# GT-RIPL/robo-vln

Measured on AMD Instinct MI355X. Metric: policy env-steps/sec (batched act()) at 256x256 RGB-D, 80-tok instr, higher is better.
Workload: dtype fp16 (range-calibrated fp16 storage and MFMA in BERT, both trunks and the cross-modal block; fp32 accumulate, fp32 recurrent state; DESIGN.md section 5); 1 GPU; BASELINE.json configs[1]: full HCM act() (hi->argmax->lo), 256x256 RGB-D, L=80, VLA N=1, LSTM-512; per_gpu_batch=64, global_batch=64, parallelism=single GPU

## Files before the change

include/hcm.h:

```cpp
#ifndef HCM_H
#define HCM_H

#include <stdint.h>

#ifdef __cplusplus
extern "C" {
#endif

typedef struct hcm_ctx* hcm_handle;

enum hcm_status {
    HCM_OK = 0,
    HCM_ERR_ARG = -1,
    HCM_ERR_STATE = -2,
    HCM_ERR_KEY = -3,
    HCM_ERR_SHAPE = -4,
    HCM_ERR_HIP = -5,
    HCM_ERR_UNSUPPORTED = -6,
    HCM_ERR_NOMEM = -7
};

enum hcm_dtype { HCM_F32 = 0, HCM_BF16 = 1, HCM_I32 = 2, HCM_I64 = 3, HCM_U8 = 4, HCM_F16 = 5 };
enum hcm_model { HCM_HIGH = 0, HCM_LOW = 1, HCM_CMA = 2 ,
                 HCM_S2S = 3  };
// ... 134 lines not shown
    int32_t struct_size;
    int32_t precision;
    int32_t max_batch;
    int32_t rgb_h, rgb_w, depth_h, depth_w;
    int32_t instr_len;
    int32_t vocab_size, embedding_size, instr_hidden;
    int32_t instr_rnn;
    int32_t bidirectional;
    int32_t rgb_encoder, depth_encoder;
    int32_t rgb_out, depth_out, depth_baseplanes;
    int32_t hidden, rnn_type;
    int32_t num_actions;
    int32_t num_sub_tasks;
    int32_t use_prev_action;
    int32_t is_bert;
    int32_t progress_monitor;
    int32_t ablate_instruction;
    int32_t ablate_depth;
    int32_t ablate_rgb;
    int32_t reserved[6];
} hcm_s2s_config;

int hcm_s2s_create(const hcm_s2s_config* cfg, hcm_handle* out);

int hcm_s2s_forward(hcm_handle h, const void* rgb, int rgb_dtype, const float* depth, const void* ids, int ids_dtype, int B, int B_instr, int L,
                    const float* h_in, const float* mask, float* out, float* stop, float* progress, float* h_out, void* stream);
int hcm_s2s_forward_seq(hcm_handle h, const void* rgb, int rgb_dtype, const float* depth, const void* ids, int ids_dtype, int T, int N, int B_instr,
                        int L, const float* h_in, const float* masks, float* out, float* stop, float* progress, float* h_out, void* stream);


int hcm_debug_enable_taps(hcm_handle h, int enable);
int hcm_debug_get_tap(hcm_handle h, const char* name, float* host_out, int64_t capacity,
                      int64_t* n_out, int64_t* shape_out);
int hcm_debug_igemm_prof(uint64_t* out8, int reset);
int hcm_debug_gemm256_prof(uint64_t* out1024, int reset);
int hcm_debug_marks(hcm_handle h, uint64_t* out256, char* names, int names_cap);

int hcm_op_conv2d(const void* x, const void* w_ohwi, const float* bias, const void* residual, void* y,
                  int dtype, int B, int H, int W, int Cin, int Cout, int KH, int KW, int stride, int pad,
                  int act, void* stream);
int hcm_op_conv2d_gn(const void* x, const void* w_ohwi, const float* gamma, const float* beta, const void* residual, void* y,
                     int dtype, int B, int H, int W, int Cin, int Cout, int KH, int KW, int stride, int pad, int groups, float eps,
                     int relu, void* stream);
int hcm_op_bottleneck_tail(const void* x, const void* w2, const float* b2, const void* w3, const float* b3, const void* identity,
                           void* y, int dtype, int B, int H, int W, int C1, int stride, void* stream);
int hcm_op_bottleneck_tail_next(const void* x, const void* w2, const float* b2, const void* w3, const float* b3, const void* identity,
                                void* y, const void* w1, const float* b1, void* o1, int dtype, int B, int H, int W, int C1, int stride,
                                int CN, void* stream);
int hcm_op_bottleneck_tail_ds(const void* x, const void* w2, const float* b2, const void* w3ds, const float* b3ds, const void* xd,
                              void* y, const void* w1, const float* b1, void* o1, int dtype, int B, int H, int W, int stride,
                              void* stream);
int hcm_op_conv2d_gn_large(const void* x, const void* w_ohwi, const float* gamma, const float* beta, const void* residual, void* y,
                           int dtype, int B, int H, int W, int Cin, int Cout, int KH, int KW, int stride, int pad, int groups, float eps,
                           int relu, void* stream);
int hcm_op_stem_conv(const void* x, int x_dtype, const void* w, const float* bias, void* y, int dtype, int B, int H, int W, int C,
                     int Cout, int KH, int KW, int stride, int pad, int K, int Kp, int rowrun, float scale, int act, void* stream);
int hcm_op_stem_conv_packed(const void* x, int x_dtype, const void* w, const float* bias, void* y, int dtype, int B, int H, int W,
                            int Cout, float scale, int act, void* scratch, void* stream);
int hcm_op_stem_conv_packed_pool(const void* x, int x_dtype, const void* w, const float* bias, void* y, int dtype, int B, int H, int W,
                                 int Cout, float scale, void* scratch, void* half_map, void* stream);
int hcm_op_stem_pool_fused(const void* x, int x_dtype, const void* w, const float* bias, void* y, int dtype, int B, int H, int W,
                           int Cout, float scale, void* scratch, void* stream);
int hcm_op_stem_pool_fused_red(const void* x, int x_dtype, const void* w, const float* bias, void* y, int dtype, int B, int H, int W,
                               int Cout, float scale, void* scratch, const void* w1, const float* b1, void* o1, void* stream);
int64_t hcm_op_stem_scratch_bytes(int B, int H, int W);
int hcm_op_depth_conv8x8s4(const float* depth, const void* w, const float* bias, void* y, int dtype, int B, int H, int act, void* scratch,
                           void* stream);
int hcm_op_simplecnn3(const float* depth, const void* w0, const float* b0, const void* w1_frag, const float* b1, const void* w2_frag, const float* b2,
                      void* y, int dtype, int B, int H, void* stream);
int hcm_op_linear(const void* x, const void* w, const float* bias, const void* residual, void* y,
                  int dtype, int M, int N, int K, int act, int out_f32, void* stream);
int hcm_op_vla_layer(const void* q, const void* I, const void* const* kv, const int* Lk, const void* const* att, void* const* out, float* const* pooled,
                     int ld_pool, const void* wo, const float* bo, const void* w1, const float* b1, const void* w2, const float* b2, const float* g1,
                     const float* be1, const float* g2, const float* be2, const int32_t* lens, int dtype, int B, int L, int d_ff, int streams,
                     void* stream);
int hcm_op_vla_layer_frag(const void* q, const void* I, const void* const* kv, const int* Lk, const void* const* att, void* const* out,
                          float* const* pooled, int ld_pool, const void* wo_frag, const float* bo, const void* w1_frag, const float* b1,
                          const void* w2_frag, const float* b2, const float* g1, const float* be1, const float* g2, const float* be2,
                          const int32_t* lens, int dtype, int B, int L, int d_ff, int streams, void* stream);
int hcm_op_linear_impl(const void* x, const void* w, const float* bias, const void* residual, void* y,
                       int dtype, int M, int N, int K, int act, int out_f32, int impl, void* stream);
int hcm_op_attention(const void* q, const void* k, const void* v, void* out, int dtype,
                     int B, int heads, int Lq, int Lk, int ldq, int ldk, int ldv, int ldo, void* stream);
int hcm_op_layernorm(const void* x, const void* residual, const float* gamma, const float* beta,
                     void* y, int dtype, int rows, int D, float eps, void* stream);
int hcm_op_pack_frag(const void* w, void* out, int dtype, int N, int K, void* stream);
int hcm_op_bert_attn_block(const void* qkv, const void* wo_frag, const float* bo, const void* residual, const float* residual32, const float* gamma,
                           const float* beta, void* y, float* y32, int dtype, int B, int L, const int32_t* lengths, float eps, void* stream);
int hcm_op_layernorm_post(const void* x, const void* residual, const float* gamma, const float* beta, const float* post, int post_rows,
                          void* y, int dtype, int rows, int D, float eps, void* stream);
int hcm_op_groupnorm(void* x_inplace, const void* residual, const float* gamma, const float* beta,
                     int dtype, int B, int HW, int C, int groups, float eps, int relu, void* stream);
int hcm_op_conv2d_gn_pool(const void* x, const void* w_ohwi, const float* gamma, const float* beta, void* y, int dtype, int B, int H, int W, int Cin,
                          int Cout, int KH, int KW, int stride, int pad, int groups, float eps, void* stream);
int hcm_op_conv2d_gn_res2(const void* x, const void* w_ohwi, const float* gamma, const float* beta, const void* x2, const void* w2_ohwi, const float* gamma2,
                          const float* beta2, void* y, int dtype, int B, int H, int W, int Cin, int Cin2, int stride2, int Cout, int groups, float eps,
                          int relu, void* stream);
int hcm_op_maxpool3x3s2(const void* x, void* y, int dtype, int B, int H, int W, int C, void* stream);
int hcm_op_val_loss(const float* logits, const float* vel, const float* stop, const int64_t* oracle_subtask, const float* corrected_actions,
                    const float* oracle_stop, float* result, int rows, int A, int num_sub_tasks, void* stream);

#ifdef __cplusplus
}
#endif
#endif
```

robo-vln_amd/_lib.py:

```python
import ctypes as C
import os

_HERE = os.path.dirname(os.path.abspath(__file__))
LIB_PATH = os.path.join(_HERE, "libhcm_dev.so" if os.environ.get("HCM_DEV_LIB", "0") not in ("", "0") else "libhcm.so")

HCM_F32, HCM_BF16, HCM_I32, HCM_I64, HCM_U8, HCM_F16 = 0, 1, 2, 3, 4, 5
HCM_HIGH, HCM_LOW, HCM_CMA, HCM_S2S = 0, 1, 2, 3
HCM_ENC_RESNET, HCM_ENC_SIMPLECNN = 0, 1
HCM_LSTM, HCM_GRU = 0, 1
(HCM_NUM_RECURRENT_LAYERS, HCM_HIDDEN_SIZE, HCM_NUM_ACTIONS, HCM_RECORD_WIDTH, HCM_WORKSPACE_BYTES,
 HCM_WEIGHT_BYTES, HCM_MAX_BATCH, HCM_GRAPH_LAUNCHES, HCM_EAGER_LAUNCHES, HCM_FP16_FALLBACK, HCM_CALIB_MAX_BERT, HCM_CALIB_MAX_DEPTH,
 HCM_CALIB_NONFINITE, HCM_CALIB_MAX_RGB, HCM_CALIB_MAX_VLA, HCM_STEP_NONFINITE, HCM_RANGE_FOLD, HCM_GATHER_JOINED) = range(18)
PRECISIONS = {"fp32": HCM_F32, "fp16": HCM_F16, "bf16": HCM_BF16}
ACT_NONE, ACT_RELU, ACT_GELU = 0, 1, 2
HCM_ACT_REUSE_INSTRUCTION = 1
HCM_ACT_HOST_FRAMES = 2
HCM_ACT_CHAIN_GRAPHS = 4

STATUS_EXC = {-1: ValueError, -2: RuntimeError, -3: KeyError, -4: ValueError, -5: RuntimeError, -6: ValueError,
              -7: MemoryError}


class HcmConfigStruct(C.Structure):
    _fields_ = [(n, C.c_int32) for n in (
# ... 4 lines not shown
        "bert_layers", "bert_hidden", "bert_heads", "bert_inter", "bert_vocab", "bert_max_pos",
        "build_high", "build_low", "use_prev_action", "ablate_instruction", "progress_monitor", "ablate_depth", "ablate_rgb")] + [("reserved", C.c_int32 * 8)]


class HcmCmaConfigStruct(C.Structure):
    _fields_ = [(n, C.c_int32) for n in (
        "struct_size", "precision", "max_batch", "rgb_h", "rgb_w", "depth_h", "depth_w", "instr_len",
        "vocab_size", "embedding_size", "instr_hidden", "bidirectional", "rgb_out", "depth_out", "depth_baseplanes",
        "hidden", "rnn_type", "num_actions", "use_prev_action", "rcm_state_encoder", "progress_monitor",
        "instr_rnn", "ablate_instruction", "ablate_depth", "ablate_rgb")] + [("reserved", C.c_int32 * 4)]


class HcmS2sConfigStruct(C.Structure):
    _fields_ = [(n, C.c_int32) for n in (
        "struct_size", "precision", "max_batch", "rgb_h", "rgb_w", "depth_h", "depth_w", "instr_len",
        "vocab_size", "embedding_size", "instr_hidden", "instr_rnn", "bidirectional", "rgb_encoder", "depth_encoder",
        "rgb_out", "depth_out", "depth_baseplanes", "hidden", "rnn_type", "num_actions", "num_sub_tasks",
        "use_prev_action", "is_bert", "progress_monitor", "ablate_instruction", "ablate_depth", "ablate_rgb")] + [("reserved", C.c_int32 * 6)]


EXPORTS = {
    "hcm_s2s_create": (C.c_int, [C.POINTER(HcmS2sConfigStruct), C.POINTER(C.c_void_p)]),
    "hcm_s2s_forward": (C.c_int, [C.c_void_p, C.c_void_p, C.c_int, C.c_void_p, C.c_void_p, C.c_int, C.c_int, C.c_int, C.c_int,
                                  C.c_void_p, C.c_void_p, C.c_void_p, C.c_void_p, C.c_void_p, C.c_void_p, C.c_void_p]),
    "hcm_s2s_forward_seq": (C.c_int, [C.c_void_p, C.c_void_p, C.c_int, C.c_void_p, C.c_void_p, C.c_int, C.c_int, C.c_int, C.c_int, C.c_int,
                                      C.c_void_p, C.c_void_p, C.c_void_p, C.c_void_p, C.c_void_p, C.c_void_p, C.c_void_p]),
    "hcm_cma_create": (C.c_int, [C.POINTER(HcmCmaConfigStruct), C.POINTER(C.c_void_p)]),
    "hcm_cma_forward": (C.c_int, [C.c_void_p, C.c_void_p, C.c_int, C.c_void_p, C.c_void_p, C.c_int, C.c_int, C.c_int,
                                  C.c_void_p, C.c_void_p, C.c_void_p, C.c_void_p, C.c_void_p, C.c_void_p]),
    "hcm_create": (C.c_int, [C.POINTER(HcmConfigStruct), C.POINTER(C.c_void_p)]),
    "hcm_load_tensor": (C.c_int, [C.c_void_p, C.c_int, C.c_char_p, C.c_void_p, C.c_int, C.POINTER(C.c_int64), C.c_int]),
    "hcm_finalize": (C.c_int, [C.c_void_p]),
    "hcm_high_forward": (C.c_int, [C.c_void_p, C.c_void_p, C.c_int, C.c_void_p, C.c_void_p, C.c_int, C.c_void_p, C.c_int, C.c_int,
                                   C.c_void_p, C.c_void_p, C.c_void_p, C.c_void_p, C.c_void_p]),
    "hcm_low_forward": (C.c_int, [C.c_void_p, C.c_void_p, C.c_int, C.c_void_p, C.c_int, C.c_void_p, C.c_void_p,
                                  C.c_void_p, C.c_void_p, C.c_void_p, C.c_void_p, C.c_void_p]),
    "hcm_high_forward_seq": (C.c_int, [C.c_void_p, C.c_void_p, C.c_int, C.c_void_p, C.c_void_p, C.c_int, C.c_void_p, C.c_int, C.c_int, C.c_int,
                                       C.c_void_p, C.c_void_p, C.c_void_p, C.c_void_p, C.c_void_p]),
    "hcm_low_forward_seq": (C.c_int, [C.c_void_p, C.c_void_p, C.c_int, C.c_void_p, C.c_int, C.c_int, C.c_void_p, C.c_void_p,
                                      C.c_void_p, C.c_void_p, C.c_void_p, C.c_void_p, C.c_void_p]),
    "hcm_val_step": (C.c_int, [C.c_void_p, C.c_void_p, C.c_int, C.c_void_p, C.c_void_p, C.c_int, C.c_void_p, C.c_int, C.c_int, C.c_int,
                               C.c_void_p, C.c_void_p, C.c_void_p, C.c_void_p, C.c_void_p, C.c_void_p, C.c_void_p, C.c_void_p, C.c_void_p,
                               C.c_void_p, C.c_void_p, C.c_void_p, C.c_void_p]),
    "hcm_act": (C.c_int, [C.c_void_p, C.c_void_p, C.c_int, C.c_void_p, C.c_void_p, C.c_int, C.c_void_p, C.c_int, C.c_int,
                          C.c_void_p, C.c_void_p, C.c_void_p, C.c_void_p, C.c_void_p, C.c_void_p, C.c_void_p]),
    "hcm_act_ex": (C.c_int, [C.c_void_p, C.c_void_p, C.c_int, C.c_void_p, C.c_void_p, C.c_int, C.c_void_p, C.c_int, C.c_int,
                             C.c_void_p, C.c_void_p, C.c_void_p, C.c_void_p, C.c_void_p, C.c_void_p, C.c_int, C.c_void_p]),
    "hcm_comm_unique_id": (C.c_int, [C.c_void_p]),
    "hcm_comm_init": (C.c_int, [C.c_void_p, C.c_void_p, C.c_int, C.c_int]),
    "hcm_comm_abort": (C.c_int, [C.c_void_p]),
    "hcm_gather_poison": (C.c_int, [C.c_void_p, C.c_int, C.c_void_p, C.c_void_p, C.c_void_p]),
    "hcm_act_gather": (C.c_int, [C.c_void_p, C.c_void_p, C.c_int, C.c_void_p, C.c_void_p, C.c_int, C.c_void_p, C.c_int, C.c_int,
                                 C.c_void_p, C.c_void_p, C.c_void_p, C.c_void_p, C.c_void_p, C.c_void_p, C.c_int, C.c_void_p, C.c_void_p]),
    "hcm_refresh_instruction": (C.c_int, [C.c_void_p, C.c_void_p, C.c_int, C.c_void_p, C.c_int, C.c_int, C.POINTER(C.c_int32), C.c_int, C.c_void_p]),
    "hcm_calibrate": (C.c_int, [C.c_void_p, C.c_void_p, C.c_int, C.c_void_p, C.c_void_p, C.c_int, C.c_int, C.c_int, C.c_void_p]),
    "hcm_release_host_weights": (C.c_int, [C.c_void_p]),
    "hcm_query": (C.c_int, [C.c_void_p, C.c_int, C.POINTER(C.c_int64)]),
    "hcm_guard_poll": (C.c_int, [C.c_void_p, C.c_void_p, C.POINTER(C.c_int64)]),
    "hcm_last_error": (C.c_char_p, [C.c_void_p]),
    "hcm_destroy": (None, [C.c_void_p]),
    "hcm_debug_enable_taps": (C.c_int, [C.c_void_p, C.c_int]),
    "hcm_debug_get_tap": (C.c_int, [C.c_void_p, C.c_char_p, C.c_void_p, C.c_int64, C.POINTER(C.c_int64), C.POINTER(C.c_int64)]),
    "hcm_debug_igemm_prof": (C.c_int, [C.POINTER(C.c_uint64), C.c_int]),
    "hcm_debug_gemm256_prof": (C.c_int, [C.POINTER(C.c_uint64), C.c_int]),
    "hcm_debug_marks": (C.c_int, [C.c_void_p, C.POINTER(C.c_uint64), C.c_char_p, C.c_int]),
    "hcm_op_conv2d": (C.c_int, [C.c_void_p] * 5 + [C.c_int] * 11 + [C.c_void_p]),
    "hcm_op_bottleneck_tail": (C.c_int, [C.c_void_p] * 7 + [C.c_int] * 6 + [C.c_void_p]),
    "hcm_op_bottleneck_tail_next": (C.c_int, [C.c_void_p] * 10 + [C.c_int] * 7 + [C.c_void_p]),
    "hcm_op_bottleneck_tail_ds": (C.c_int, [C.c_void_p] * 10 + [C.c_int] * 5 + [C.c_void_p]),
    "hcm_op_conv2d_gn": (C.c_int, [C.c_void_p] * 6 + [C.c_int] * 11 + [C.c_float, C.c_int, C.c_void_p]),
    "hcm_op_conv2d_gn_large": (C.c_int, [C.c_void_p] * 6 + [C.c_int] * 11 + [C.c_float, C.c_int, C.c_void_p]),
    "hcm_op_stem_conv": (C.c_int, [C.c_void_p, C.c_int, C.c_void_p, C.c_void_p, C.c_void_p] + [C.c_int] * 13 + [C.c_float, C.c_int, C.c_void_p]),
    "hcm_op_stem_conv_packed": (C.c_int, [C.c_void_p, C.c_int, C.c_void_p, C.c_void_p, C.c_void_p] + [C.c_int] * 5 + [C.c_float, C.c_int, C.c_void_p, C.c_void_p]),
    "hcm_op_stem_pool_fused": (C.c_int, [C.c_void_p, C.c_int, C.c_void_p, C.c_void_p, C.c_void_p] + [C.c_int] * 5 + [C.c_float, C.c_void_p, C.c_void_p]),
    "hcm_op_stem_pool_fused_red": (C.c_int, [C.c_void_p, C.c_int, C.c_void_p, C.c_void_p, C.c_void_p] + [C.c_int] * 5 + [C.c_float] + [C.c_void_p] * 5),
    "hcm_op_stem_conv_packed_pool": (C.c_int, [C.c_void_p, C.c_int, C.c_void_p, C.c_void_p, C.c_void_p] + [C.c_int] * 5 + [C.c_float, C.c_void_p, C.c_void_p, C.c_void_p]),
    "hcm_op_depth_conv8x8s4": (C.c_int, [C.c_void_p] * 4 + [C.c_int] * 4 + [C.c_void_p, C.c_void_p]),
    "hcm_op_stem_scratch_bytes": (C.c_int64, [C.c_int] * 3),
    "hcm_op_linear": (C.c_int, [C.c_void_p] * 5 + [C.c_int] * 6 + [C.c_void_p]),
    "hcm_op_linear_impl": (C.c_int, [C.c_void_p] * 5 + [C.c_int] * 7 + [C.c_void_p]),
    "hcm_op_vla_layer": (C.c_int, [C.c_void_p] * 7 + [C.c_int] + [C.c_void_p] * 11 + [C.c_int] * 5 + [C.c_void_p]),
    "hcm_op_vla_layer_frag": (C.c_int, [C.c_void_p] * 7 + [C.c_int] + [C.c_void_p] * 11 + [C.c_int] * 5 + [C.c_void_p]),
    "hcm_op_attention": (C.c_int, [C.c_void_p] * 4 + [C.c_int] * 9 + [C.c_void_p]),
    "hcm_op_simplecnn3": (C.c_int, [C.c_void_p] * 8 + [C.c_int] * 3 + [C.c_void_p]),
    "hcm_op_pack_frag": (C.c_int, [C.c_void_p, C.c_void_p, C.c_int, C.c_int, C.c_int, C.c_void_p]),
    "hcm_op_bert_attn_block": (C.c_int, [C.c_void_p] * 9 + [C.c_int] * 3 + [C.c_void_p, C.c_float, C.c_void_p]),
    "hcm_op_layernorm": (C.c_int, [C.c_void_p] * 5 + [C.c_int] * 3 + [C.c_float, C.c_void_p]),
    "hcm_op_layernorm_post": (C.c_int, [C.c_void_p] * 5 + [C.c_int, C.c_void_p] + [C.c_int] * 3 + [C.c_float, C.c_void_p]),
    "hcm_op_groupnorm": (C.c_int, [C.c_void_p] * 4 + [C.c_int] * 5 + [C.c_float, C.c_int, C.c_void_p]),
    "hcm_op_conv2d_gn_pool": (C.c_int, [C.c_void_p] * 5 + [C.c_int] * 11 + [C.c_float, C.c_void_p]),
    "hcm_op_conv2d_gn_res2": (C.c_int, [C.c_void_p] * 9 + [C.c_int] * 9 + [C.c_float, C.c_int, C.c_void_p]),
    "hcm_op_val_loss": (C.c_int, [C.c_void_p] * 7 + [C.c_int] * 3 + [C.c_void_p]),
    "hcm_op_maxpool3x3s2": (C.c_int, [C.c_void_p] * 2 + [C.c_int] * 5 + [C.c_void_p]),
}

_lib = None


def lib():
    global _lib
    if _lib is None:
        if not os.path.exists(LIB_PATH):
            raise RuntimeError(f"{LIB_PATH} is missing: build it with `python -c 'import __graft_entry__ as g; g.build()'` "
                               "(the HIP library is the only compute path; there is no CPU fallback)")
        l = C.CDLL(LIB_PATH)
        for name, (res, args) in EXPORTS.items():
            fn = getattr(l, name)
            fn.restype = res
            fn.argtypes = args
        _lib = l
    return _lib


def last_error(handle=None):
    msg = lib().hcm_last_error(handle)
    return msg.decode() if msg else ""


def check(rc, handle=None):
    if rc == 0:
        return
    msg = lib().hcm_last_error(handle)
    msg = msg.decode() if msg else f"libhcm error {rc}"
    raise STATUS_EXC.get(rc, RuntimeError)(msg)
```

robo-vln_amd/csrc/api.cpp:

```cpp
#include <chrono>
#include <cmath>
#include <cstdlib>
#include <cstring>
#include <stdexcept>
#include <string>

#include "model.h"

namespace hcm {
void build_spec_high(hcm_ctx* ctx);
void build_spec_low(hcm_ctx* ctx);
void prepare_high(hcm_ctx* ctx);
void prepare_low(hcm_ctx* ctx);
void build_spec_cma(hcm_ctx* ctx);
void prepare_cma(hcm_ctx* ctx);
void run_refresh_instruction(hcm_ctx* ctx, const void* ids, int ids_dt, int B, const int32_t* idx, int n);
void run_cma(hcm_ctx* ctx, const void* rgb, int rgb_dt, const float* depth, const void* ids, int ids_dt, int B, const float* h_in,
             const float* mask, float* out, float* stop, float* h_out);
void build_spec_s2s(hcm_ctx* ctx);
void prepare_s2s(hcm_ctx* ctx);
void run_s2s(hcm_ctx* ctx, const void* rgb, int rgb_dt, const float* depth, const void* ids, int ids_dt, int B, int Bi, const float* h_in,
             const float* mask, float* out, float* stop, float* progress, float* h_out, int T = 1);
void comm_destroy(hcm_ctx* ctx);
void run_step(hcm_ctx* ctx, bool do_hi, bool do_lo, const void* rgb, int rgb_dt, const float* depth, const void* ids, int ids_dt,
// ... 1239 lines not shown
static void* op_scratch(size_t bytes) {
    static void* buf = nullptr;
    static size_t cap = 0;
    if (bytes > cap) {
        if (buf) { (void)hipDeviceSynchronize(); (void)hipFree(buf); }
        if (hipMalloc(&buf, bytes) != hipSuccess) { buf = nullptr; cap = 0; return nullptr; }
        cap = bytes;
    }
    return buf;
}
int hcm_op_linear(const void* x, const void* w, const float* bias, const void* residual, void* y, int dtype, int M, int N, int K,
                  int act, int out_f32, void* stream) {
    {
        int S = splitk_slices(M, N, K, dtype == HCM_F32 ? 4 : 8, residual != nullptr);
        static const int force_s = dev_env("HCM_SPLITK_FORCE") ? atoi(dev_env("HCM_SPLITK_FORCE")) : 0;
        if (force_s > 0 && !residual && K % (force_s * 64) == 0) S = force_s;
        if (S > 1) {
            float* part = (float*)op_scratch((size_t)S * M * N * 4);
            if (!part) return HCM_ERR_NOMEM;
            const int Ks = K / S;
            IGemm g;
            g.x = x; g.w = w; g.y = part;
            g.B = M; g.Cin = Ks; g.xC = K; g.M = M; g.N = N; g.K = Ks; g.Kp = K; g.ldy = N; g.ldr = N; g.act = ACT_NONE; g.out_f32 = 1;
            g.groups = S; g.g_x = Ks; g.g_w = Ks; g.g_b = 0; g.g_y = (long long)M * N;
            int rc = op_rc(launch_igemm(g, op_dt(dtype), (hipStream_t)stream));
            if (rc != HCM_OK) return rc;
            return op_rc(launch_splitk_reduce(part, bias, y, op_dt(dtype), S, M, N, N, act, out_f32, (hipStream_t)stream));
        }
    }
    IGemm g;
    g.x = x; g.w = w; g.bias = bias; g.res = residual; g.y = y;
    g.B = M; g.Cin = K; g.xC = K; g.M = M; g.N = N; g.K = K; g.Kp = K; g.ldy = N; g.ldr = N; g.act = act; g.out_f32 = out_f32;
    return op_rc(launch_igemm(g, op_dt(dtype), (hipStream_t)stream));
}
int hcm_op_linear_impl(const void* x, const void* w, const float* bias, const void* residual, void* y, int dtype, int M, int N, int K,
                       int act, int out_f32, int impl, void* stream) {
    IGemm g;
    g.x = x; g.w = w; g.bias = bias; g.res = residual; g.y = y;
    g.B = M; g.Cin = K; g.xC = K; g.M = M; g.N = N; g.K = K; g.Kp = K; g.ldy = N; g.ldr = N; g.act = act; g.out_f32 = out_f32;
    g.impl = impl;
    return op_rc(launch_igemm(g, op_dt(dtype), (hipStream_t)stream));
}
static int op_vla_layer(const void* q, const void* I, const void* const* kv, const int* Lk, const void* const* att, void* const* out, float* const* pooled,
                        int ld_pool, const void* wo, const float* bo, const void* w1, const float* b1, const void* w2, const float* b2, const float* g1,
                        const float* be1, const float* g2, const float* be2, const int32_t* lens, int dtype, int B, int L, int d_ff, int streams,
                        void* stream, int wfrag);
int hcm_op_vla_layer(const void* q, const void* I, const void* const* kv, const int* Lk, const void* const* att, void* const* out, float* const* pooled,
                     int ld_pool, const void* wo, const float* bo, const void* w1, const float* b1, const void* w2, const float* b2, const float* g1,
                     const float* be1, const float* g2, const float* be2, const int32_t* lens, int dtype, int B, int L, int d_ff, int streams,
                     void* stream) {
    return op_vla_layer(q, I, kv, Lk, att, out, pooled, ld_pool, wo, bo, w1, b1, w2, b2, g1, be1, g2, be2, lens, dtype, B, L, d_ff, streams, stream, 0);
}
int hcm_op_vla_layer_frag(const void* q, const void* I, const void* const* kv, const int* Lk, const void* const* att, void* const* out,
                          float* const* pooled, int ld_pool, const void* wo_frag, const float* bo, const void* w1_frag, const float* b1,
                          const void* w2_frag, const float* b2, const float* g1, const float* be1, const float* g2, const float* be2,
                          const int32_t* lens, int dtype, int B, int L, int d_ff, int streams, void* stream) {
    return op_vla_layer(q, I, kv, Lk, att, out, pooled, ld_pool, wo_frag, bo, w1_frag, b1, w2_frag, b2, g1, be1, g2, be2, lens, dtype, B, L, d_ff, streams,
                        stream, 1);
}
static int op_vla_layer(const void* q, const void* I, const void* const* kv, const int* Lk, const void* const* att, void* const* out, float* const* pooled,
                        int ld_pool, const void* wo, const float* bo, const void* w1, const float* b1, const void* w2, const float* b2, const float* g1,
                        const float* be1, const float* g2, const float* be2, const int32_t* lens, int dtype, int B, int L, int d_ff, int streams,
                        void* stream, int wfrag) {
    if (!I || !out || !wo || !w1 || !w2 || !bo || !b1 || !b2 || !g1 || !be1 || !g2 || !be2 || streams < 1 || streams > 2) return HCM_ERR_ARG;
    if (!vla_post_ok(op_dt(dtype), 256, 4, d_ff)) return HCM_ERR_ARG;
    VlaPost p;
    p.q = q; p.I = I; p.B = B; p.L = L; p.d_ff = d_ff; p.lens = lens; p.streams = streams; p.ld_pool = ld_pool;
    p.wo = wo; p.bo = bo; p.w1 = w1; p.b1 = b1; p.w2 = w2; p.b2 = b2; p.g1 = g1; p.be1 = be1; p.g2 = g2; p.be2 = be2;
    p.wfrag = wfrag;
    p.fuse_att = kv != nullptr;
    if (p.fuse_att && (!q || !Lk)) return HCM_ERR_ARG;
    if (!p.fuse_att && !att) return HCM_ERR_ARG;
    for (int s = 0; s < streams; ++s) {
        if (p.fuse_att) { p.kv[s] = kv[s]; p.Lk[s] = Lk[s]; } else p.att[s] = att[s];
        p.out[s] = out[s];
        p.pooled[s] = pooled ? pooled[s] : nullptr;
    }
    return op_rc(launch_vla_post(p, op_dt(dtype), (hipStream_t)stream));
}
int hcm_op_attention(const void* q, const void* k, const void* v, void* out, int dtype, int B, int heads, int Lq, int Lk, int ldq,
                     int ldk, int ldv, int ldo, void* stream) {
    return op_rc(launch_attention(q, k, v, out, op_dt(dtype), B, heads, Lq, Lk, ldq, ldk, ldv, ldo, B, (hipStream_t)stream));
}
int hcm_op_layernorm(const void* x, const void* residual, const float* gamma, const float* beta, void* y, int dtype, int rows,
                     int D, float eps, void* stream) {
    return op_rc(launch_layernorm(x, residual, gamma, beta, nullptr, 0, y, op_dt(dtype), rows, D, eps, (hipStream_t)stream));
}
int hcm_op_simplecnn3(const float* depth, const void* w0, const float* b0, const void* w1_frag, const float* b1, const void* w2_frag, const float* b2,
                      void* y, int dtype, int B, int H, void* stream) {
    return op_rc(launch_simplecnn3(depth, w0, b0, w1_frag, b1, w2_frag, b2, y, op_dt(dtype), B, H, (hipStream_t)stream));
}
int hcm_op_pack_frag(const void* w, void* out, int dtype, int N, int K, void* stream) {
    return op_rc(launch_pack_frag(w, out, op_dt(dtype), N, K, (hipStream_t)stream));
}
int hcm_op_bert_attn_block(const void* qkv, const void* wo, const float* bo, const void* residual, const float* residual32, const float* gamma,
                           const float* beta, void* y, float* y32, int dtype, int B, int L, const int32_t* lengths, float eps, void* stream) {
    return op_rc(launch_bert_attn_block(qkv, 2304, wo, bo, residual, residual32, gamma, beta, y, y32, op_dt(dtype), B, L, lengths, eps, (hipStream_t)stream));
}
int hcm_op_layernorm_post(const void* x, const void* residual, const float* gamma, const float* beta, const float* post, int post_rows,
                          void* y, int dtype, int rows, int D, float eps, void* stream) {
    return op_rc(launch_layernorm(x, residual, gamma, beta, post, post_rows, y, op_dt(dtype), rows, D, eps, (hipStream_t)stream));
}
int hcm_op_groupnorm(void* x_inplace, const void* residual, const float* gamma, const float* beta, int dtype, int B, int HW, int C,
                     int groups, float eps, int relu, void* stream) {
    static float* scratch = nullptr;
    static size_t scratch_floats = 0;
    const size_t need = gn_stats_floats(B, HW, groups);
    if (need > scratch_floats) {
        if (scratch) { (void)hipDeviceSynchronize(); (void)hipFree(scratch); }
        if (hipMalloc((void**)&scratch, need * 4) != hipSuccess) return HCM_ERR_NOMEM;
        scratch_floats = need;
    }
    return op_rc(launch_groupnorm(x_inplace, residual, gamma, beta, scratch, op_dt(dtype), B, HW, C, groups, eps, relu, (hipStream_t)stream));
}
int hcm_op_conv2d_gn_large(const void* x, const void* w_ohwi, const float* gamma, const float* beta, const void* residual, void* y,
                           int dtype, int B, int H, int W, int Cin, int Cout, int KH, int KW, int stride, int pad, int groups, float eps,
                           int relu, void* stream) {
    if (groups < 1 || Cout % groups) return HCM_ERR_ARG;
    const int Ho = (H + 2 * pad - KH) / stride + 1, Wo = (W + 2 * pad - KW) / stride + 1, hw = Ho * Wo, dt = op_dt(dtype);
    if (!groupnorm_apply_ok(dt, hw, Cout, groups)) return HCM_ERR_ARG;
    static float* scratch = nullptr;
    static size_t scratch_floats = 0;
    const size_t need = gn_stats_floats(B, hw, groups);
    if (need > scratch_floats) {
        if (scratch) { (void)hipDeviceSynchronize(); (void)hipFree(scratch); }
        if (hipMalloc((void**)&scratch, need * 4) != hipSuccess) return HCM_ERR_NOMEM;
        scratch_floats = need;
    }
    IGemm g;
    g.x = x; g.w = w_ohwi; g.y = y;
    g.B = B; g.H = H; g.W = W; g.Cin = Cin; g.xC = Cin; g.Ho = Ho; g.Wo = Wo;
    g.KH = KH; g.KW = KW; g.stride = stride; g.pad = pad;
    g.M = B * hw; g.N = Cout; g.K = KH * KW * Cin; g.Kp = g.K; g.ldy = Cout; g.ldr = Cout; g.act = ACT_NONE;
    g.cs_part = scratch; g.cs_cg = Cout / groups; g.cs_hw = hw; g.cs_G = groups;
    int rc = op_rc(launch_igemm(g, dt, (hipStream_t)stream));
    if (rc != HCM_OK) return rc;
    return op_rc(launch_groupnorm_apply(y, residual, gamma, beta, scratch, hw / 64, dt, B, hw, Cout, groups, eps, relu, (hipStream_t)stream));
}
int hcm_op_conv2d_gn_pool(const void* x, const void* w_ohwi, const float* gamma, const float* beta, void* y, int dtype, int B, int H, int W, int Cin,
                          int Cout, int KH, int KW, int stride, int pad, int groups, float eps, void* stream) {
    if (groups < 1 || Cout % groups) return HCM_ERR_ARG;
    const int Ho = (H + 2 * pad - KH) / stride + 1, Wo = (W + 2 * pad - KW) / stride + 1, hw = Ho * Wo, dt = op_dt(dtype);
    if (!groupnorm_apply_ok(dt, hw, Cout, groups) || !maxpool_gn_ok(dt, Cout, groups)) return HCM_ERR_ARG;
    const size_t stats_bytes = (gn_stats_floats(B, hw, groups) * 4 + 255) / 256 * 256, map_bytes = (size_t)B * hw * Cout * 2;
    char* sc = (char*)op_scratch(stats_bytes + map_bytes);
    if (!sc) return HCM_ERR_NOMEM;
    float* stats = (float*)sc;
    void* raw = sc + stats_bytes;
    IGemm g;
    g.x = x; g.w = w_ohwi; g.y = raw;
    g.B = B; g.H = H; g.W = W; g.Cin = Cin; g.xC = Cin; g.Ho = Ho; g.Wo = Wo;
    g.KH = KH; g.KW = KW; g.stride = stride; g.pad = pad;
    g.M = B * hw; g.N = Cout; g.K = KH * KW * Cin; g.Kp = g.K; g.ldy = Cout; g.ldr = Cout; g.act = ACT_NONE;
    g.cs_part = stats; g.cs_cg = Cout / groups; g.cs_hw = hw; g.cs_G = groups;
    int rc = op_rc(launch_igemm(g, dt, (hipStream_t)stream));
    if (rc != HCM_OK) return rc;
    const int Hp = (Ho + 2 - 3) / 2 + 1, Wp = (Wo + 2 - 3) / 2 + 1;
    return op_rc(launch_maxpool3x3s2_gn(raw, y, gamma, beta, stats, hw / 64, eps, groups, dt, B, Ho, Wo, Cout, Hp, Wp, (hipStream_t)stream));
}
int hcm_op_conv2d_gn_res2(const void* x, const void* w_ohwi, const float* gamma, const float* beta, const void* x2, const void* w2_ohwi, const float* gamma2,
                          const float* beta2, void* y, int dtype, int B, int H, int W, int Cin, int Cin2, int stride2, int Cout, int groups, float eps,
                          int relu, void* stream) {
    if (groups < 1 || Cout % groups || stride2 < 1) return HCM_ERR_ARG;
    const int hw = H * W, dt = op_dt(dtype);
    if (!groupnorm_apply_ok(dt, hw, Cout, groups)) return HCM_ERR_ARG;
    const size_t stats_bytes = (gn_stats_floats(B, hw, groups) * 4 + 255) / 256 * 256, map_bytes = (size_t)B * hw * Cout * 2;
// ... 33 lines not shown
```

robo-vln_amd/csrc/attention.hip:

```cpp
#include <cstdlib>
#include "kernels.h"
#include "dev.h"

namespace hcm {

template <typename T>
__global__ __launch_bounds__(256) void attention_kernel(const T* __restrict__ q, const T* __restrict__ k, const T* __restrict__ v,
                                                        T* __restrict__ out, int heads, int Lq, int Lk0, int ldq, int ldk,
                                                        int ldv, int ldo, int q_batch_mod, int KC, const int* __restrict__ klens) {
    constexpr int CH = Tr<T>::CH;
    constexpr int D = 64;
    extern __shared__ __attribute__((aligned(16))) char smem_att[];
    float* Ks = reinterpret_cast<float*>(smem_att);
    float* Vs = Ks + (size_t)KC * D;

    const int b = blockIdx.x / heads;
    const int h = blockIdx.x % heads;
    const int bq = b % q_batch_mod;
    const int tid = threadIdx.x;
    int Lk = Lk0;
    if (klens) { Lk = klens[b]; Lk = Lk < 1 ? 1 : Lk > Lk0 ? Lk0 : Lk; }

    const int part = tid & 3;
    {
// ... 133 lines not shown
        for (int j = 0; j < 8; ++j) {
            T t;
            t.v = (uint16_t)(w[j >> 1] >> ((j & 1) * 16));
            Vt[(size_t)(c * 8 + j) * vstride + row] = t;
        }
    }
    __syncthreads();

    for (int qt = wave; qt < QT; qt += nwaves) {
        if (qt != wave) {
            int qrow = qt * 16 + fr;
            if (qrow >= Lq) qrow = Lq - 1;
            const T* qp = q + ((size_t)bq * Lq + qrow) * ldq + h * D;
            q0 = *reinterpret_cast<const uint4*>(qp + fg * 8);
            q1 = *reinterpret_cast<const uint4*>(qp + 32 + fg * 8);
        }

        f32x4_t sc[MAXKT];
        float mx = -3.0e38f;
#pragma unroll
        for (int t = 0; t < MAXKT; ++t) {
            sc[t] = (f32x4_t){0.f, 0.f, 0.f, 0.f};
            if (t < 2 * KT2) {
                const int r = t * 16 + fr;
                const uint4 k0 = *reinterpret_cast<const uint4*>(Ks + r * 128 + (((0 + fg) ^ (r & 7)) << 4));
                const uint4 k1 = *reinterpret_cast<const uint4*>(Ks + r * 128 + (((4 + fg) ^ (r & 7)) << 4));
                sc[t] = AttMma<T>::run(k0, q0, sc[t]);
                sc[t] = AttMma<T>::run(k1, q1, sc[t]);
#pragma unroll
                for (int e = 0; e < 4; ++e) {
                    const int key = t * 16 + fg * 4 + e;
                    const float sv = key < Lk ? sc[t][e] * 0.125f : -3.0e38f;
                    sc[t][e] = sv;
                    mx = fmaxf(mx, sv);
                }
            }
        }
        mx = fmaxf(mx, __shfl_xor(mx, 16, 64));
        mx = fmaxf(mx, __shfl_xor(mx, 32, 64));
        float sum = 0.f;
#pragma unroll
        for (int t = 0; t < MAXKT; ++t)
            if (t < 2 * KT2) {
#pragma unroll
                for (int e = 0; e < 4; ++e) {
                    const float pv = __expf(sc[t][e] - mx);
                    sc[t][e] = pv;
                    sum += pv;
                }
            }
        sum += __shfl_xor(sum, 16, 64);
        sum += __shfl_xor(sum, 32, 64);

        f32x4_t o[4];
#pragma unroll
        for (int dtile = 0; dtile < 4; ++dtile) o[dtile] = (f32x4_t){0.f, 0.f, 0.f, 0.f};
#pragma unroll
        for (int c2 = 0; c2 < MAXKT / 2; ++c2)
            if (c2 < KT2) {
                uint4 pa;
                pa.x = pack2<T>(sc[2 * c2][0], sc[2 * c2][1]);
                pa.y = pack2<T>(sc[2 * c2][2], sc[2 * c2][3]);
                pa.z = pack2<T>(sc[2 * c2 + 1][0], sc[2 * c2 + 1][1]);
                pa.w = pack2<T>(sc[2 * c2 + 1][2], sc[2 * c2 + 1][3]);
#pragma unroll
                for (int dtile = 0; dtile < 4; ++dtile) {
                    const T* vr = Vt + (size_t)(dtile * 16 + fr) * vstride + c2 * 32 + fg * 4;
                    const uint2 lo = *reinterpret_cast<const uint2*>(vr);
                    const uint2 hi = *reinterpret_cast<const uint2*>(vr + 16);
                    const uint4 vb = make_uint4(lo.x, lo.y, hi.x, hi.y);
                    o[dtile] = AttMma<T>::run(pa, vb, o[dtile]);
                }
            }
        const float inv = 1.0f / sum;
#pragma unroll
        for (int e = 0; e < 4; ++e) {
            const float inv_q = __shfl(inv, fg * 4 + e, 64);
            const int qi = qt * 16 + fg * 4 + e;
            if (qi < Lq) {
                T* op = out + ((size_t)b * Lq + qi) * ldo + h * D + fr;
#pragma unroll
                for (int dtile = 0; dtile < 4; ++dtile) Tr<T>::st(op + dtile * 16, o[dtile][e] * inv_q);
            }
        }
    }
}

hipError_t launch_attention(const void* q, const void* k, const void* v, void* out, int dt, int B, int heads, int Lq,
                            int Lk, int ldq, int ldk, int ldv, int ldo, int q_batch_mod, hipStream_t s, const int* klens) {
    constexpr int KC_MAX = 256;
    const int KC = Lk < KC_MAX ? Lk : KC_MAX;
    const size_t lds = (size_t)KC * 64 * sizeof(float) * 2;
    if (Lk < 1 || Lq < 1) return hipErrorInvalidValue;
    const int CH = dt_chunk(dt);
    if ((ldq % CH) || (ldk % CH) || (ldv % CH) || (ldo % CH)) return hipErrorInvalidValue;
    if (q_batch_mod <= 0) q_batch_mod = B;
    static DeviceOnce attr_once;
    if (attr_once.need()) {
        (void)hipFuncSetAttribute(reinterpret_cast<const void*>(attention_kernel<bf16>), hipFuncAttributeMaxDynamicSharedMemorySize, 160 * 1024);
        (void)hipFuncSetAttribute(reinterpret_cast<const void*>(attention_kernel<f16>), hipFuncAttributeMaxDynamicSharedMemorySize, 160 * 1024);
        (void)hipFuncSetAttribute(reinterpret_cast<const void*>(attention_kernel<float>), hipFuncAttributeMaxDynamicSharedMemorySize, 160 * 1024);
        (void)hipFuncSetAttribute(reinterpret_cast<const void*>(attention_mfma_kernel<bf16, 16>), hipFuncAttributeMaxDynamicSharedMemorySize, 160 * 1024);
        (void)hipFuncSetAttribute(reinterpret_cast<const void*>(attention_mfma_kernel<f16, 16>), hipFuncAttributeMaxDynamicSharedMemorySize, 160 * 1024);
        (void)hipFuncSetAttribute(reinterpret_cast<const void*>(attention_mfma_kernel<bf16, 32>), hipFuncAttributeMaxDynamicSharedMemorySize, 160 * 1024);
        (void)hipFuncSetAttribute(reinterpret_cast<const void*>(attention_mfma_kernel<f16, 32>), hipFuncAttributeMaxDynamicSharedMemorySize, 160 * 1024);
        attr_once.done();
    }
    static const char* valu = dev_env("HCM_ATT_VALU");
    if ((dt == DT_BF16 || dt == DT_F16) && Lk <= 512 && !(valu && atoi(valu))) {
        const int Lkp = (Lk + 31) / 32 * 32;
        const size_t lds2 = (size_t)Lkp * 128 + (size_t)64 * (Lkp + 4) * 2;
        static const bool w4 = dev_env("HCM_ATT_W4") != nullptr;
        const int qtiles = (Lq + 15) / 16;
        const int threads = w4 ? 256 : 64 * (qtiles < 4 ? 4 : qtiles > 8 ? 8 : qtiles);
#define LM(T, KT) hipLaunchKernelGGL((attention_mfma_kernel<T, KT>), dim3(B * heads), dim3(threads), lds2, s, (const T*)q, (const T*)k, (const T*)v, (T*)out, heads, Lq, Lk, ldq, ldk, ldv, ldo, q_batch_mod, klens)
        if (Lk <= 160) { if (dt == DT_BF16) LM(bf16, 10); else LM(f16, 10); }
        else if (Lk <= 256) { if (dt == DT_BF16) LM(bf16, 16); else LM(f16, 16); }
        else { if (dt == DT_BF16) LM(bf16, 32); else LM(f16, 32); }
#undef LM
        return hipGetLastError();
    }
#define LA(T) hipLaunchKernelGGL(attention_kernel<T>, dim3(B * heads, (Lq + 63) / 64), dim3(256), lds, s, (const T*)q, (const T*)k, (const T*)v, (T*)out, heads, Lq, Lk, ldq, ldk, ldv, ldo, q_batch_mod, KC, klens)
    if (dt == DT_BF16) LA(bf16); else if (dt == DT_F16) LA(f16); else if (dt == DT_F32) LA(float); else return hipErrorInvalidValue;
#undef LA
    return hipGetLastError();
}

}
```

Measured before the change: 15110 env-steps/s.

## Add wide attention kernel with swizzled LDS, transpose reads and coalesced output stores

Adds a new MFMA attention kernel, now the default (the old one stays behind HCM_ATT_V1). It stages K and V with batched 16-byte loads into XOR-swizzled LDS, reads V through ds_read_tr16 transpose loads, and writes output through a per-wave LDS tile after a DPP lane exchange, so global stores become coalesced 16-byte rows. The aim is to cut LDS bank conflicts and uncoalesced global stores in BERT and cross-modal attention. It uses more LDS per block, which may lower occupancy. It also adds an attention_ex API entry point that exposes q_batch_mod and klens.

```diff
diff --git a/include/hcm.h b/include/hcm.h
--- a/include/hcm.h
+++ b/include/hcm.h
@@ -240,6 +240,8 @@
                        int dtype, int M, int N, int K, int act, int out_f32, int impl, void* stream);
 int hcm_op_attention(const void* q, const void* k, const void* v, void* out, int dtype,
                      int B, int heads, int Lq, int Lk, int ldq, int ldk, int ldv, int ldo, void* stream);
+int hcm_op_attention_ex(const void* q, const void* k, const void* v, void* out, int dtype, int B, int heads, int Lq, int Lk,
+                        int ldq, int ldk, int ldv, int ldo, int q_batch_mod, const int32_t* klens, void* stream);
 int hcm_op_layernorm(const void* x, const void* residual, const float* gamma, const float* beta,
                      void* y, int dtype, int rows, int D, float eps, void* stream);
 int hcm_op_pack_frag(const void* w, void* out, int dtype, int N, int K, void* stream);
diff --git a/robo-vln_amd/_lib.py b/robo-vln_amd/_lib.py
--- a/robo-vln_amd/_lib.py
+++ b/robo-vln_amd/_lib.py
@@ -110,6 +110,7 @@
     "hcm_op_vla_layer": (C.c_int, [C.c_void_p] * 7 + [C.c_int] + [C.c_void_p] * 11 + [C.c_int] * 5 + [C.c_void_p]),
     "hcm_op_vla_layer_frag": (C.c_int, [C.c_void_p] * 7 + [C.c_int] + [C.c_void_p] * 11 + [C.c_int] * 5 + [C.c_void_p]),
     "hcm_op_attention": (C.c_int, [C.c_void_p] * 4 + [C.c_int] * 9 + [C.c_void_p]),
+    "hcm_op_attention_ex": (C.c_int, [C.c_void_p] * 4 + [C.c_int] * 10 + [C.c_void_p, C.c_void_p]),
     "hcm_op_simplecnn3": (C.c_int, [C.c_void_p] * 8 + [C.c_int] * 3 + [C.c_void_p]),
     "hcm_op_pack_frag": (C.c_int, [C.c_void_p, C.c_void_p, C.c_int, C.c_int, C.c_int, C.c_void_p]),
     "hcm_op_bert_attn_block": (C.c_int, [C.c_void_p] * 9 + [C.c_int] * 3 + [C.c_void_p, C.c_float, C.c_void_p]),
diff --git a/robo-vln_amd/csrc/api.cpp b/robo-vln_amd/csrc/api.cpp
--- a/robo-vln_amd/csrc/api.cpp
+++ b/robo-vln_amd/csrc/api.cpp
@@ -1345,6 +1345,10 @@
                      int ldk, int ldv, int ldo, void* stream) {
     return op_rc(launch_attention(q, k, v, out, op_dt(dtype), B, heads, Lq, Lk, ldq, ldk, ldv, ldo, B, (hipStream_t)stream));
 }
+int hcm_op_attention_ex(const void* q, const void* k, const void* v, void* out, int dtype, int B, int heads, int Lq, int Lk, int ldq,
+                        int ldk, int ldv, int ldo, int q_batch_mod, const int32_t* klens, void* stream) {
+    return op_rc(launch_attention(q, k, v, out, op_dt(dtype), B, heads, Lq, Lk, ldq, ldk, ldv, ldo, q_batch_mod, (hipStream_t)stream, klens));
+}
 int hcm_op_layernorm(const void* x, const void* residual, const float* gamma, const float* beta, void* y, int dtype, int rows,
                      int D, float eps, void* stream) {
     return op_rc(launch_layernorm(x, residual, gamma, beta, nullptr, 0, y, op_dt(dtype), rows, D, eps, (hipStream_t)stream));
diff --git a/robo-vln_amd/csrc/attention.hip b/robo-vln_amd/csrc/attention.hip
--- a/robo-vln_amd/csrc/attention.hip
+++ b/robo-vln_amd/csrc/attention.hip
@@ -239,6 +239,180 @@
 #pragma unroll
                 for (int dtile = 0; dtile < 4; ++dtile) Tr<T>::st(op + dtile * 16, o[dtile][e] * inv_q);
             }
+        }
+    }
+}
+
+typedef short att_s16x4 __attribute__((ext_vector_type(4)));
+constexpr int ATT_SB = 4;
+constexpr int ATT_OROW = 144;
+constexpr int ATT_OTILE = 16 * ATT_OROW;
+
+__device__ __forceinline__ uint2 lds_read_tr16(const char* p) {
+    const att_s16x4 r = __builtin_amdgcn_ds_read_tr16_b64_v4i16((__attribute__((address_space(3))) att_s16x4*)p);
+    return __builtin_bit_cast(uint2, r);
+}
+__device__ __forceinline__ void wave_lds_handoff() {
+    __builtin_amdgcn_fence(__ATOMIC_RELEASE, "wavefront");
+    __builtin_amdgcn_wave_barrier();
+    __builtin_amdgcn_fence(__ATOMIC_ACQUIRE, "wavefront");
+}
+
+template <typename T, int MAXKT>
+__global__ __launch_bounds__(512) void attention_wide_kernel(const T* __restrict__ q, const T* __restrict__ k, const T* __restrict__ v,
+                                                             T* __restrict__ out, int heads, int Lq, int Lk0, int ldq, int ldk,
+                                                             int ldv, int ldo, int q_batch_mod, const int* __restrict__ klens) {
+    int Lk = Lk0;
+    if (klens) { Lk = klens[blockIdx.x / heads]; Lk = Lk < 1 ? 1 : Lk > Lk0 ? Lk0 : Lk; }
+    constexpr int D = 64;
+    extern __shared__ __attribute__((aligned(16))) char smem_att[];
+    const int KT2 = (Lk + 31) / 32;
+    const int Lkp = KT2 * 32;
+    char* Ks = smem_att;
+    char* Vs = smem_att + (size_t)Lkp * 128;
+
+    const int b = blockIdx.x / heads;
+    const int h = blockIdx.x % heads;
+    const int bq = b % q_batch_mod;
+    const int tid = threadIdx.x;
+    const int lane = tid & 63;
+    const int wave = tid >> 6;
+    const int nthreads = blockDim.x, nwaves = nthreads >> 6;
+    char* Ot = smem_att + (size_t)Lkp * 256 + wave * ATT_OTILE;
+
+    const int fr = lane & 15, fg = lane >> 4;
+    const int QT = (Lq + 15) / 16;
+    uint4 q0 = make_uint4(0, 0, 0, 0), q1 = q0;
+    if (wave < QT) {
+        int qrow = wave * 16 + fr;
+        if (qrow >= Lq) qrow = Lq - 1;
+        const T* qp = q + ((size_t)bq * Lq + qrow) * ldq + h * D;
+        q0 = *reinterpret_cast<const uint4*>(qp + fg * 8);
+        q1 = *reinterpret_cast<const uint4*>(qp + 32 + fg * 8);
+    }
+    const int nchunks = Lkp * 8;
+    for (int e0 = tid; e0 < nchunks; e0 += nthreads * ATT_SB) {
+        uint4 kv[ATT_SB], vv[ATT_SB];
+#pragma unroll
+        for (int i = 0; i < ATT_SB; ++i) {
+            const int e = e0 + i * nthreads;
+            const int row = e >> 3, c = e & 7;
+            kv[i] = make_uint4(0, 0, 0, 0);
+            vv[i] = make_uint4(0, 0, 0, 0);
+            if (row < Lk) {
+                kv[i] = *reinterpret_cast<const uint4*>(k + ((size_t)b * Lk0 + row) * ldk + h * D + c * 8);
+                vv[i] = *reinterpret_cast<const uint4*>(v + ((size_t)b * Lk0 + row) * ldv + h * D + c * 8);
+            }
+        }
+#pragma unroll
+        for (int i = 0; i < ATT_SB; ++i) {
+            const int e = e0 + i * nthreads;
+            const int row = e >> 3, c = e & 7;
+            if (e < nchunks) {
+                const int off = row * 128 + ((c ^ (row & 7)) << 4);
+                *reinterpret_cast<uint4*>(Ks + off) = kv[i];
+                *reinterpret_cast<uint4*>(Vs + off) = vv[i];
+            }
+        }
+    }
+    __syncthreads();
+
+    const int tq = fr >> 2, tp = fr & 3, trow = fg * 4 + tq;
+    int voff[4];
+#pragma unroll
+    for (int dtile = 0; dtile < 4; ++dtile) voff[dtile] = trow * 128 + (((2 * dtile + (tp >> 1)) ^ (trow & 7)) << 4) + (tp & 1) * 8;
+    const bool odd = lane & 1;
+
+    for (int qt = wave; qt < QT; qt += nwaves) {
+        if (qt != wave) {
+            int qrow = qt * 16 + fr;
+            if (qrow >= Lq) qrow = Lq - 1;
+            const T* qp = q + ((size_t)bq * Lq + qrow) * ldq + h * D;
+            q0 = *reinterpret_cast<const uint4*>(qp + fg * 8);
+            q1 = *reinterpret_cast<const uint4*>(qp + 32 + fg * 8);
+        }
+
+        f32x4_t sc[MAXKT];
+        float mx = -3.0e38f;
+#pragma unroll
+        for (int t = 0; t < MAXKT; ++t) {
+            sc[t] = (f32x4_t){0.f, 0.f, 0.f, 0.f};
+            if (t < 2 * KT2) {
+                const int r = t * 16 + fr;
+                const uint4 k0 = *reinterpret_cast<const uint4*>(Ks + r * 128 + (((0 + fg) ^ (r & 7)) << 4));
+                const uint4 k1 = *reinterpret_cast<const uint4*>(Ks + r * 128 + (((4 + fg) ^ (r & 7)) << 4));
+                sc[t] = AttMma<T>::run(k0, q0, sc[t]);
+                sc[t] = AttMma<T>::run(k1, q1, sc[t]);
+#pragma unroll
+                for (int e = 0; e < 4; ++e) {
+                    const int key = t * 16 + fg * 4 + e;
+                    const float sv = key < Lk ? sc[t][e] * 0.125f : -3.0e38f;
+                    sc[t][e] = sv;
+                    mx = fmaxf(mx, sv);
+                }
+            }
+        }
+        mx = fmaxf(mx, __shfl_xor(mx, 16, 64));
+        mx = fmaxf(mx, __shfl_xor(mx, 32, 64));
+        float sum = 0.f;
+#pragma unroll
+        for (int t = 0; t < MAXKT; ++t)
+            if (t < 2 * KT2) {
+#pragma unroll
+                for (int e = 0; e < 4; ++e) {
+                    const float pv = __expf(sc[t][e] - mx);
+                    sc[t][e] = pv;
+                    sum += pv;
+                }
+            }
+        sum += __shfl_xor(sum, 16, 64);
+        sum += __shfl_xor(sum, 32, 64);
+
+        f32x4_t o[4];
+#pragma unroll
+        for (int dtile = 0; dtile < 4; ++dtile) o[dtile] = (f32x4_t){0.f, 0.f, 0.f, 0.f};
+#pragma unroll
+        for (int c2 = 0; c2 < MAXKT / 2; ++c2)
+            if (c2 < KT2) {
+                uint4 pa;
+                pa.x = pack2<T>(sc[2 * c2][0], sc[2 * c2][1]);
+                pa.y = pack2<T>(sc[2 * c2][2], sc[2 * c2][3]);
+                pa.z = pack2<T>(sc[2 * c2 + 1][0], sc[2 * c2 + 1][1]);
+                pa.w = pack2<T>(sc[2 * c2 + 1][2], sc[2 * c2 + 1][3]);
+#pragma unroll
+                for (int dtile = 0; dtile < 4; ++dtile) {
+                    const char* vr = Vs + c2 * 4096 + voff[dtile];
+                    const uint2 lo = lds_read_tr16(vr);
+                    const uint2 hi = lds_read_tr16(vr + 2048);
+                    const uint4 vb = make_uint4(lo.x, lo.y, hi.x, hi.y);
+                    o[dtile] = AttMma<T>::run(pa, vb, o[dtile]);
+                }
+            }
+        const float inv = 1.0f / sum;
+        float inv_q[4];
+#pragma unroll
+        for (int e = 0; e < 4; ++e) inv_q[e] = __shfl(inv, fg * 4 + e, 64);
+        wave_lds_handoff();
+#pragma unroll
+        for (int dtile = 0; dtile < 4; ++dtile) {
+            const uint32_t w01 = pack2<T>(o[dtile][0] * inv_q[0], o[dtile][1] * inv_q[1]);
+            const uint32_t w23 = pack2<T>(o[dtile][2] * inv_q[2], o[dtile][3] * inv_q[3]);
+            const uint32_t give = odd ? w01 : w23;
+            const uint32_t got = (uint32_t)__builtin_amdgcn_mov_dpp((int)give, 0xB1, 0xF, 0xF, true);
+            const uint32_t a = odd ? got : w01, c = odd ? w23 : got;
+            const uint32_t r0 = (a & 0xFFFFu) | (c << 16);
+            const uint32_t r1 = (a >> 16) | (c & 0xFFFF0000u);
+            char* op = Ot + (fg * 4 + (odd ? 2 : 0)) * ATT_OROW + dtile * 32 + (fr & ~1) * 2;
+            *reinterpret_cast<uint32_t*>(op) = r0;
+            *reinterpret_cast<uint32_t*>(op + ATT_OROW) = r1;
+        }
+        wave_lds_handoff();
+#pragma unroll
+        for (int s2 = 0; s2 < 2; ++s2) {
+            const int row = s2 * 8 + (lane >> 3), c = lane & 7;
+            const uint4 val = *reinterpret_cast<const uint4*>(Ot + row * ATT_OROW + c * 16);
+            const int qi = qt * 16 + row;
+            if (qi < Lq) *reinterpret_cast<uint4*>(out + ((size_t)b * Lq + qi) * ldo + h * D + c * 8) = val;
         }
     }
 }
@@ -261,6 +435,10 @@
         (void)hipFuncSetAttribute(reinterpret_cast<const void*>(attention_mfma_kernel<f16, 16>), hipFuncAttributeMaxDynamicSharedMemorySize, 160 * 1024);
         (void)hipFuncSetAttribute(reinterpret_cast<const void*>(attention_mfma_kernel<bf16, 32>), hipFuncAttributeMaxDynamicSharedMemorySize, 160 * 1024);
         (void)hipFuncSetAttribute(reinterpret_cast<const void*>(attention_mfma_kernel<f16, 32>), hipFuncAttributeMaxDynamicSharedMemorySize, 160 * 1024);
+        (void)hipFuncSetAttribute(reinterpret_cast<const void*>(attention_wide_kernel<bf16, 16>), hipFuncAttributeMaxDynamicSharedMemorySize, 160 * 1024);
+        (void)hipFuncSetAttribute(reinterpret_cast<const void*>(attention_wide_kernel<f16, 16>), hipFuncAttributeMaxDynamicSharedMemorySize, 160 * 1024);
+        (void)hipFuncSetAttribute(reinterpret_cast<const void*>(attention_wide_kernel<bf16, 32>), hipFuncAttributeMaxDynamicSharedMemorySize, 160 * 1024);
+        (void)hipFuncSetAttribute(reinterpret_cast<const void*>(attention_wide_kernel<f16, 32>), hipFuncAttributeMaxDynamicSharedMemorySize, 160 * 1024);
         attr_once.done();
     }
     static const char* valu = dev_env("HCM_ATT_VALU");
@@ -270,7 +448,10 @@
         static const bool w4 = dev_env("HCM_ATT_W4") != nullptr;
         const int qtiles = (Lq + 15) / 16;
         const int threads = w4 ? 256 : 64 * (qtiles < 4 ? 4 : qtiles > 8 ? 8 : qtiles);
-#define LM(T, KT) hipLaunchKernelGGL((attention_mfma_kernel<T, KT>), dim3(B * heads), dim3(threads), lds2, s, (const T*)q, (const T*)k, (const T*)v, (T*)out, heads, Lq, Lk, ldq, ldk, ldv, ldo, q_batch_mod, klens)
+        static const bool v1 = dev_env("HCM_ATT_V1") != nullptr;
+        const size_t lds3 = (size_t)Lkp * 256 + (size_t)(threads / 64) * ATT_OTILE;
+#define LM(T, KT) do { if (v1) hipLaunchKernelGGL((attention_mfma_kernel<T, KT>), dim3(B * heads), dim3(threads), lds2, s, (const T*)q, (const T*)k, (const T*)v, (T*)out, heads, Lq, Lk, ldq, ldk, ldv, ldo, q_batch_mod, klens); \
+                       else hipLaunchKernelGGL((attention_wide_kernel<T, KT>), dim3(B * heads), dim3(threads), lds3, s, (const T*)q, (const T*)k, (const T*)v, (T*)out, heads, Lq, Lk, ldq, ldk, ldv, ldo, q_batch_mod, klens); } while (0)
         if (Lk <= 160) { if (dt == DT_BF16) LM(bf16, 10); else LM(f16, 10); }
         else if (Lk <= 256) { if (dt == DT_BF16) LM(bf16, 16); else LM(f16, 16); }
         else { if (dt == DT_BF16) LM(bf16, 32); else LM(f16, 32); }
```

Result: no change. 15130 env-steps/s, median of 6 (+0.2%).
